# supernomad/quantum

Measured on AMD Instinct MI355X. Metric: AES-256-GCM seal+unseal GiB/s (device-resident packets) at 1/2/4/8 MI355X, higher is better.
Workload: dtype u8

## Files before the change

### quantum_amd/csrc/gcm_kernels.hip

```cpp
#include <hip/hip_runtime.h>
#include <stdint.h>

#include <algorithm>

#include "gcm_internal.h"

namespace qgcm {

typedef __attribute__((address_space(3))) uint32_t lds_u32;
typedef uint32_t u32x4 __attribute__((ext_vector_type(4)));
typedef __attribute__((address_space(3))) u32x4 lds_u128;

struct __attribute__((aligned(4))) W4 {
    uint32_t x, y, z, w;
};

#ifndef QGCM_NT_DATA
#define QGCM_NT_DATA 0
#endif
typedef uint32_t u32x4u __attribute__((ext_vector_type(4), aligned(4)));
__device__ __forceinline__ W4 load_block(const W4 *p) {
    if constexpr ((QGCM_NT_DATA & 1) != 0) {
        const u32x4u v = __builtin_nontemporal_load(reinterpret_cast<const u32x4u *>(p));
        return W4{v.x, v.y, v.z, v.w};
// ... 127 lines not shown
    const uint32_t t2 = xor3(t.t0(s2, 0), t.t1(s3, 1), rot16(xor3(t.t0(s0, 2), t.t1(s1, 3), k.rr6)));
    const uint32_t t3 = xor3(t.t0(s3, 0), t.t1(s0, 1), rot16(xor3(t.t0(s1, 2), t.t1(s2, 3), k.rr7)));
    c.U0 = t.t1(t1, 1) ^ rot16(xor3(t.t0(t2, 2), t.t1(t3, 3), k.rr8));
    c.U1 = xor3(t.t0(t1, 0), t.t1(t2, 1), rot16(t.t0(t3, 2))) ^ k.rk9;
    c.U2 = xor3(t.t0(t2, 0), t.t1(t3, 1), rot16(t.t1(t1, 3))) ^ k.rk10;
    c.U3 = t.t0(t3, 0) ^ rot16(xor3(t.t0(t1, 2), t.t1(t2, 3), k.rr11));
}
template <class A>
__device__ __forceinline__ void ctr_setup(Ctr &c, uint32_t n0, uint32_t n1, uint32_t n2, uint32_t ctr_hi,
                                          const Keys &k, const A &t) {
    ctr_setup(c, n0, n1, n2, ctr_hi, setup_keys(k), t);
}
__device__ __forceinline__ void ctr_setup(Ctr &c, uint32_t n0, uint32_t n1, uint32_t n2, uint32_t ctr_hi,
                                          const Keys &k, uint32_t lb) {
    ctr_setup(c, n0, n1, n2, ctr_hi, k, TT0{lb, 0});
}

template <class A, uint32_t kB>
__device__ __forceinline__ void ctr_block_t(const Ctr &c, uint32_t lo, const Keys &k, const A &t, uint32_t &s0,
                                            uint32_t &s1, uint32_t &s2, uint32_t &s3) {
    const uint32_t x = lo ^ c.x3;
    const uint32_t t0 = c.K0 ^ rot16(lds32(((x << 8) | t.lb) + kB + 128u));
    s0 = c.U0 ^ t.t0(t0, 0);
    s1 = c.U1 ^ rot16(t.t1(t0, 3));
    s2 = c.U2 ^ rot16(t.t0(t0, 2));
    s3 = c.U3 ^ t.t1(t0, 1);
#pragma unroll
    for (int r = 3; r < 14; ++r) round_full(s0, s1, s2, s3, k, r, t);
    round_last(s0, s1, s2, s3, k, t);
}
__device__ __forceinline__ void ctr_block(const Ctr &c, uint32_t lo, const Keys &k, uint32_t lb, uint32_t &s0,
                                          uint32_t &s1, uint32_t &s2, uint32_t &s3) {
    ctr_block_t<TT0, 0>(c, lo, k, TT0{lb, 0}, s0, s1, s2, s3);
}

template <bool kFence>
__device__ __forceinline__ void ghash_mul(uint32_t &y0, uint32_t &y1, uint32_t &y2, uint32_t &y3, uint32_t gb);

struct Tab2 {
    Keys kk;
    TT<0, true> t;
    __device__ __forceinline__ void setup(Ctr &c, uint32_t n0, uint32_t n1, uint32_t n2, uint32_t hi) const {
        ctr_setup(c, n0, n1, n2, hi, kk, t);
    }
    __device__ __forceinline__ void block(const Ctr &c, uint32_t lo, uint32_t &k0, uint32_t &k1, uint32_t &k2,
                                          uint32_t &k3) const {
        ctr_block_t<TT<0, true>, 0>(c, lo, kk, t, k0, k1, k2, k3);
    }
    __device__ __forceinline__ void ghash(uint32_t &y0, uint32_t &y1, uint32_t &y2, uint32_t &y3, uint32_t gb) const {
        ghash_mul<true>(y0, y1, y2, y3, gb);
    }
};

constexpr uint32_t kG5Windows = 26;
constexpr uint32_t kG5Bytes = kG5Windows * 512;

template <int kI>
__device__ __forceinline__ uint32_t g5_addr(const uint32_t (&y)[4], uint32_t mf8) {
    constexpr int p = 5 * kI, w = p >> 5, o = p & 31;
    uint32_t x;
    if constexpr (o > 27 && w < 3)
        x = __builtin_amdgcn_alignbit(y[w + 1], y[w], o - 3);
    else if constexpr (o > 3)
        x = y[w] >> (o - 3);
    else if constexpr (o < 3)
        x = y[w] << (3 - o);
    else
        x = y[w];
    return x & mf8;
}

template <int kLo, int kHi>
__device__ __forceinline__ void g5_chunk(const uint32_t (&y)[4], uint32_t mf8, uint32_t &a0, uint32_t &a1,
                                         uint32_t &a2, uint32_t &a3) {
    if constexpr (kLo < kHi) {
        if constexpr (QGCM_GH_PRIO > 0) __builtin_amdgcn_s_setprio(QGCM_GH_PRIO);
        const uint32_t x = g5_addr<kLo>(y, mf8);
        const u32x2 h0 = lds64(x + kLo * 512u), h1 = lds64(x + kLo * 512u + 256u);
        if constexpr (kLo + 1 < kHi) {
            const uint32_t x2 = g5_addr<kLo + 1>(y, mf8);
            const u32x2 l0 = lds64(x2 + (kLo + 1) * 512u), l1 = lds64(x2 + (kLo + 1) * 512u + 256u);
            if constexpr (QGCM_GH_PRIO > 0) __builtin_amdgcn_s_setprio(0);
            a0 = xor3(a0, h0.x, l0.x);
            a1 = xor3(a1, h0.y, l0.y);
            a2 = xor3(a2, h1.x, l1.x);
            a3 = xor3(a3, h1.y, l1.y);
            g5_chunk<kLo + 2, kHi>(y, mf8, a0, a1, a2, a3);
        } else {
            if constexpr (QGCM_GH_PRIO > 0) __builtin_amdgcn_s_setprio(0);
            a0 ^= h0.x;
            a1 ^= h0.y;
            a2 ^= h1.x;
            a3 ^= h1.y;
        }
    }
}

__device__ __forceinline__ void ghash_mul5(uint32_t &y0, uint32_t &y1, uint32_t &y2, uint32_t &y3, uint32_t mf8) {
    const uint32_t y[4] = {y0, y1, y2, y3};
    uint32_t a0 = 0, a1 = 0, a2 = 0, a3 = 0;
    g5_chunk<0, 7>(y, mf8, a0, a1, a2, a3);
    asm volatile("" : "+v"(a0), "+v"(a1), "+v"(a2), "+v"(a3)::"memory");
    g5_chunk<7, 13>(y, mf8, a0, a1, a2, a3);
    asm volatile("" : "+v"(a0), "+v"(a1), "+v"(a2), "+v"(a3)::"memory");
    g5_chunk<13, 20>(y, mf8, a0, a1, a2, a3);
    asm volatile("" : "+v"(a0), "+v"(a1), "+v"(a2), "+v"(a3)::"memory");
    g5_chunk<20, 26>(y, mf8, a0, a1, a2, a3);
    y0 = a0;
    y1 = a1;
    y2 = a2;
    y3 = a3;
}

__device__ __forceinline__ void g5_fill(const uint4 *__restrict__ comb4, uint32_t tid, uint32_t nthreads) {
    for (uint32_t e = tid; e < kG5Windows * 32u; e += nthreads) {
        const uint32_t i = e >> 5, v = e & 31u;
        uint4 c[5];
#pragma unroll
        for (uint32_t j = 0; j < 5; ++j) {
            const uint32_t t = 5 * i + j, tt = t < 128u ? t : 127u;
            const uint32_t vv = (((v >> j) & 1u) && t < 128u) ? (1u << (tt & 3u)) : 0u;
            c[j] = comb4[16u * (2u * (tt >> 3) + ((tt & 7u) < 4u ? 1u : 0u)) + vv];
        }
        uint32_t a0 = 0, a1 = 0, a2 = 0, a3 = 0;
#pragma unroll
        for (uint32_t j = 0; j < 5; ++j) {
            a0 ^= c[j].x;
            a1 ^= c[j].y;
            a2 ^= c[j].z;
            a3 ^= c[j].w;
        }
        *(lds_u64 *)(size_t)(512u * i + 8u * v) = u32x2{a0, a1};
        *(lds_u64 *)(size_t)(512u * i + 256u + 8u * v) = u32x2{a2, a3};
    }
}

struct Tab2F {
    Keys kk;
    TT<kG5Bytes, true> t;
    uint32_t mf8;
    __device__ __forceinline__ void setup(Ctr &c, uint32_t n0, uint32_t n1, uint32_t n2, uint32_t hi) const {
        ctr_setup(c, n0, n1, n2, hi, kk, t);
    }
    __device__ __forceinline__ void block(const Ctr &c, uint32_t lo, uint32_t &k0, uint32_t &k1, uint32_t &k2,
                                          uint32_t &k3) const {
        ctr_block_t<TT<kG5Bytes, true>, kG5Bytes>(c, lo, kk, t, k0, k1, k2, k3);
    }
    __device__ __forceinline__ void ghash(uint32_t &y0, uint32_t &y1, uint32_t &y2, uint32_t &y3, uint32_t) const {
        ghash_mul5(y0, y1, y2, y3, mf8);
    }
};

__device__ __forceinline__ uint32_t vreg(uint32_t x) {
    asm volatile("" : "+v"(x));
    return x;
}

template <bool kFence = true>
__device__ __forceinline__ void ghash_mul(uint32_t &y0, uint32_t &y1, uint32_t &y2, uint32_t &y3, uint32_t gb) {
    uint32_t a0 = 0, a1 = 0, a2 = 0, a3 = 0;
    const uint32_t yw[4] = {y0, y1, y2, y3};
#pragma unroll
    for (int w = 0; w < 4; ++w) {
        const uint32_t hi = yw[w] & 0xf0f0f0f0u;
        const uint32_t lo = (yw[w] << 4) & 0xf0f0f0f0u;
#pragma unroll
        for (int k = 0; k < 4; ++k) {
            const int j = 4 * w + k;
            const uint4 th = lds128(perm(gb, hi, 0x0c060500u | k) + (2 * j) * 256);
            const uint4 tl = lds128(perm(gb, lo, 0x0c060500u | k) + (2 * j + 1) * 256);
            a0 = xor3(a0, th.x, tl.x);
            a1 = xor3(a1, th.y, tl.y);
            a2 = xor3(a2, th.z, tl.z);
            a3 = xor3(a3, th.w, tl.w);
        }
        if constexpr (kFence) asm volatile("" : "+v"(a0), "+v"(a1), "+v"(a2), "+v"(a3)::"memory");
    }
    y0 = a0;
    y1 = a1;
    y2 = a2;
    y3 = a3;
}

__device__ __forceinline__ void ghash_mul_global(uint32_t &y0, uint32_t &y1, uint32_t &y2, uint32_t &y3,
                                                 const uint4 *__restrict__ T) {
    uint32_t a0 = 0, a1 = 0, a2 = 0, a3 = 0;
    const uint32_t yw[4] = {y0, y1, y2, y3};
    const char *base = reinterpret_cast<const char *>(T);
#pragma unroll
    for (int w = 0; w < 4; ++w) {
#pragma unroll
        for (int k = 0; k < 4; ++k) {
            const int j = 4 * w + k;
            const uint32_t oh = (yw[w] >> (8 * k)) & 0xf0u;
            const uint32_t ol = ((yw[w] >> (8 * k)) & 0x0fu) << 4;
            const uint4 th = *reinterpret_cast<const uint4 *>(base + (2 * j) * 256 + oh);
            const uint4 tl = *reinterpret_cast<const uint4 *>(base + (2 * j + 1) * 256 + ol);
            a0 = xor3(a0, th.x, tl.x);
            a1 = xor3(a1, th.y, tl.y);
            a2 = xor3(a2, th.z, tl.z);
            a3 = xor3(a3, th.w, tl.w);
        }
        asm volatile("" : "+v"(a0), "+v"(a1), "+v"(a2), "+v"(a3)::"memory");
    }
    y0 = a0;
    y1 = a1;
    y2 = a2;
    y3 = a3;
}

__device__ __forceinline__ void ghash_lenblock_global(uint32_t aad_len, uint32_t L, const uint4 *__restrict__ T,
                                                      uint32_t &y0, uint32_t &y1, uint32_t &y2, uint32_t &y3) {
    const char *base = reinterpret_cast<const char *>(T);
    const uint32_t w1 = bswap(aad_len * 8u), w3 = bswap(L * 8u);
    const uint32_t v[5] = {w1 >> 24, w3, w3 >> 8, w3 >> 16, w3 >> 24};
    const int j[5] = {7, 12, 13, 14, 15};
    uint32_t a0 = 0, a1 = 0, a2 = 0, a3 = 0;
#pragma unroll
    for (int i = 0; i < 5; ++i) {
        const uint4 th = *reinterpret_cast<const uint4 *>(base + (2 * j[i]) * 256 + (v[i] & 0xf0u));
        const uint4 tl = *reinterpret_cast<const uint4 *>(base + (2 * j[i] + 1) * 256 + ((v[i] & 0x0fu) << 4));
        a0 = xor3(a0, th.x, tl.x);
        a1 = xor3(a1, th.y, tl.y);
        a2 = xor3(a2, th.z, tl.z);
        a3 = xor3(a3, th.w, tl.w);
    }
    y0 = a0;
    y1 = a1;
    y2 = a2;
    y3 = a3;
}

__device__ __forceinline__ uint32_t sel4(uint32_t q, uint32_t a, uint32_t b, uint32_t c, uint32_t d) {
    return q == 0 ? a : (q == 1 ? b : (q == 2 ? c : d));
}
__device__ __forceinline__ uint32_t lowmask(uint32_t s) { return s ? (0xffffffffu >> (32 - 8 * s)) : 0u; }
__device__ __forceinline__ void store_bytes(uint8_t *p, uint32_t v, uint32_t nbytes) {
    if (nbytes > 0) p[0] = (uint8_t)v;
    if (nbytes > 1) p[1] = (uint8_t)(v >> 8);
    if (nbytes > 2) p[2] = (uint8_t)(v >> 16);
}
__device__ __forceinline__ uint32_t load_bytes(const uint8_t *p, uint32_t nbytes) {
    uint32_t v = 0;
    if (nbytes > 0) v |= p[0];
    if (nbytes > 1) v |= (uint32_t)p[1] << 8;
    if (nbytes > 2) v |= (uint32_t)p[2] << 16;
    return v;
}


__device__ __forceinline__ void read_tail(const uint8_t *data, uint32_t L, uint32_t &g0, uint32_t &g1, uint32_t &g2,
                                          uint32_t &g3, uint32_t &n0, uint32_t &n1, uint32_t &n2) {
    const uint32_t s = L & 3u;
    const uint32_t *t = reinterpret_cast<const uint32_t *>(data + (L & ~3u));
    const uint32_t w0 = t[0], w1 = t[1], w2 = t[2], w3 = t[3], w4 = t[4], w5 = t[5], w6 = t[6];
    const uint32_t w7 = load_bytes(data + (L & ~3u) + 28, s);
    g0 = __builtin_amdgcn_alignbyte(w1, w0, s);
    g1 = __builtin_amdgcn_alignbyte(w2, w1, s);
    g2 = __builtin_amdgcn_alignbyte(w3, w2, s);
    g3 = __builtin_amdgcn_alignbyte(w4, w3, s);
    n0 = __builtin_amdgcn_alignbyte(w5, w4, s);
    n1 = __builtin_amdgcn_alignbyte(w6, w5, s);
    n2 = __builtin_amdgcn_alignbyte(w7, w6, s);
}

__device__ __forceinline__ void read_nonce(const uint8_t *data, uint32_t L, uint32_t &n0, uint32_t &n1, uint32_t &n2) {
    const uint32_t s = L & 3u;
    const uint32_t *t = reinterpret_cast<const uint32_t *>(data + (L & ~3u));
    const uint32_t w4 = t[4], w5 = t[5], w6 = t[6];
    const uint32_t w7 = load_bytes(data + (L & ~3u) + 28, s);
    n0 = __builtin_amdgcn_alignbyte(w5, w4, s);
    n1 = __builtin_amdgcn_alignbyte(w6, w5, s);
    n2 = __builtin_amdgcn_alignbyte(w7, w6, s);
}
__device__ __forceinline__ void read_tag(const uint8_t *data, uint32_t L, uint32_t &g0, uint32_t &g1, uint32_t &g2,
                                         uint32_t &g3) {
    const uint32_t s = L & 3u;
    const uint32_t *t = reinterpret_cast<const uint32_t *>(data + (L & ~3u));
    const uint32_t w0 = t[0], w1 = t[1], w2 = t[2], w3 = t[3], w4 = t[4];
    g0 = __builtin_amdgcn_alignbyte(w1, w0, s);
    g1 = __builtin_amdgcn_alignbyte(w2, w1, s);
    g2 = __builtin_amdgcn_alignbyte(w3, w2, s);
    g3 = __builtin_amdgcn_alignbyte(w4, w3, s);
}

__device__ __forceinline__ uint32_t funnel(uint32_t hi, uint32_t lo, uint32_t sh) {
    return (uint32_t)((((uint64_t)hi << 32) | lo) >> sh);
}
__device__ __forceinline__ void write_tail(uint8_t *data, uint32_t L, uint32_t g0, uint32_t g1, uint32_t g2,
                                           uint32_t g3, uint32_t n0, uint32_t n1, uint32_t n2, uint32_t prefix) {
    const uint32_t s = L & 3u;
    uint32_t *t = reinterpret_cast<uint32_t *>(data + (L & ~3u));
    const uint32_t sh = 32 - 8 * s;
    t[0] = (uint32_t)((((uint64_t)g0 << 32) | ((uint64_t)prefix << sh)) >> sh);
    t[1] = funnel(g1, g0, sh);
    t[2] = funnel(g2, g1, sh);
    t[3] = funnel(g3, g2, sh);
    t[4] = funnel(n0, g3, sh);
    t[5] = funnel(n1, n0, sh);
    t[6] = funnel(n2, n1, sh);
    if (s) store_bytes(data + (L & ~3u) + 28, n2 >> sh, s);
}

__device__ __forceinline__ uint32_t quad_xor(uint32_t v) {
    v ^= (uint32_t)__builtin_amdgcn_mov_dpp((int)v, 0xB1, 0xf, 0xf, false);
    v ^= (uint32_t)__builtin_amdgcn_mov_dpp((int)v, 0x4E, 0xf, 0xf, false);
    return v;
}

template <bool kSeal, class Eng>
__device__ __forceinline__ void quad_packet(const Batch &b, const Eng &eng, uint32_t pkt, uint64_t off, uint32_t L,
                                            uint32_t wkey, uint32_t m, uint32_t gH4) {
    const uint4 *Hg = b.gh_table + (size_t)wkey * kGhEntries;
    uint8_t *raw = b.arena + off;
    uint8_t *data = raw + 4;

    uint32_t g0 = 0, g1 = 0, g2 = 0, g3 = 0, n0, n1, n2;
    if (kSeal && b.nonces) {
        const uint32_t *np = reinterpret_cast<const uint32_t *>(b.nonces + 12ull * pkt);
        n0 = np[0];
        n1 = np[1];
        n2 = np[2];
    } else {
        read_nonce(data, L, n0, n1, n2);
    }
    const uint32_t nfull = L >> 4, r = L & 15u;
    const uint32_t d = nfull + (r ? 1u : 0u);

    uint32_t z0 = 0, z1 = 0, z2 = 0, z3 = 0;
    if (m == 3 && b.aad_len)
        z0 = *reinterpret_cast<const uint32_t *>(raw) & (b.aad_len >= 4 ? 0xffffffffu : lowmask(b.aad_len));
    int blast = -1;

    uint32_t e0 = 0, e1 = 0, e2 = 0, e3 = 0;
    uint32_t prefix = 0;
    {
    Ctr cc;
    uint32_t hi = 0;
    eng.setup(cc, n0, n1, n2, 0);
    for (uint32_t bi = m; bi < nfull; bi += 4) {
        const uint32_t ctr = bi + 2;
        if ((ctr >> 8) != hi) {
            hi = ctr >> 8;
            eng.setup(cc, n0, n1, n2, hi);
        }
        W4 *p = reinterpret_cast<W4 *>(data + 16u * bi);
        const W4 in = load_block(p);
        uint32_t k0, k1, k2, k3;
        eng.block(cc, ctr & 0xffu, k0, k1, k2, k3);
        const W4 out = {in.x ^ k0, in.y ^ k1, in.z ^ k2, in.w ^ k3};
        store_block(p, out);
        const W4 &c = kSeal ? out : in;
        eng.ghash(z0, z1, z2, z3, gH4);
        z0 ^= c.x;
        z1 ^= c.y;
        z2 ^= c.z;
        z3 ^= c.w;
        blast = (int)bi;
    }
    const bool part = r && (nfull & 3u) == m;
    if (part || m == (d & 3u)) {
        const uint32_t ctr = part ? nfull + 2 : 1u;
        if ((ctr >> 8) != hi) {
            hi = ctr >> 8;
            eng.setup(cc, n0, n1, n2, hi);
        }
        uint32_t k0, k1, k2, k3;
        eng.block(cc, ctr & 0xffu, k0, k1, k2, k3);
        if (part) {
            uint8_t *blk = data + 16u * nfull;
            const W4 in = *reinterpret_cast<const W4 *>(blk);
            const uint32_t q = r >> 2, sb = r & 3u;
            const uint32_t o0 = in.x ^ k0, o1 = in.y ^ k1, o2 = in.z ^ k2, o3 = in.w ^ k3;
            uint32_t *bw = reinterpret_cast<uint32_t *>(blk);
            if (q > 0) bw[0] = o0;
            if (q > 1) bw[1] = o1;
            if (q > 2) bw[2] = o2;
            const uint32_t oq = sel4(q, o0, o1, o2, o3) & lowmask(sb);
            W4 c = kSeal ? W4{o0, o1, o2, o3} : in;
            if (kSeal)
                prefix = oq;
            else
                store_bytes(blk + 4 * q, oq, sb);
            c.x &= q > 0 ? 0xffffffffu : lowmask(sb);
            c.y &= q > 1 ? 0xffffffffu : (q == 1 ? lowmask(sb) : 0u);
            c.z &= q > 2 ? 0xffffffffu : (q == 2 ? lowmask(sb) : 0u);
            c.w &= q == 3 ? lowmask(sb) : 0u;
            eng.ghash(z0, z1, z2, z3, gH4);
            z0 ^= c.x;
            z1 ^= c.y;
            z2 ^= c.z;
            z3 ^= c.w;
            blast = (int)nfull;
        } else {
            e0 = k0;
            e1 = k1;
            e2 = k2;
            e3 = k3;
        }
    }
    }
    {
        const uint32_t em = d + 1u - (uint32_t)blast;
        const uint32_t tsel = em == 2 ? kGhH2 : em == 3 ? kGhH3 : em == 4 ? kGhH4 : kGhH5;
        ghash_mul_global(z0, z1, z2, z3, Hg + tsel);
        uint32_t l0, l1, l2, l3;
        ghash_lenblock_global(b.aad_len, L, Hg, l0, l1, l2, l3);
        z0 = quad_xor(z0) ^ l0;
        z1 = quad_xor(z1) ^ l1;
        z2 = quad_xor(z2) ^ l2;
        z3 = quad_xor(z3) ^ l3;
    }
    e0 = quad_xor(e0);
    e1 = quad_xor(e1);
    e2 = quad_xor(e2);
    e3 = quad_xor(e3);
    const uint32_t t0 = z0 ^ e0, t1 = z1 ^ e1, t2 = z2 ^ e2, t3 = z3 ^ e3;
    const uint32_t owner = r ? (nfull & 3u) : 0u;
    if (kSeal) {
        if (m == owner) {
            write_tail(data, L, t0, t1, t2, t3, n0, n1, n2, prefix);
            if (b.status) b.status[pkt] = 1;
        }
    } else {
        read_tag(data, L, g0, g1, g2, g3);
        const bool ok = ((t0 ^ g0) | (t1 ^ g1) | (t2 ^ g2) | (t3 ^ g3)) == 0;
        if (!ok) {
            for (uint32_t bi = m; bi < nfull; bi += 4) {
                const W4 zz = {0, 0, 0, 0};
                *reinterpret_cast<W4 *>(data + 16u * bi) = zz;
            }
            if (r && m == owner) {
                uint32_t *bw = reinterpret_cast<uint32_t *>(data + 16u * nfull);
                for (uint32_t w = 0; w < (r >> 2); ++w) bw[w] = 0;
                store_bytes(data + 16u * nfull + (r & ~3u), 0, r & 3u);
            }
        }
        if (b.status && m == 0) b.status[pkt] = ok ? 1 : 0;
    }
}

#ifndef QGCM_TILE_POOL
#define QGCM_TILE_POOL 4
#endif
#ifndef QGCM_TAIL_EIGHTHS
#define QGCM_TAIL_EIGHTHS 4
#endif
constexpr uint32_t kPoolCtr = kG5Bytes + kTeBytes;

#ifdef QGCM_QUAD_STATS
__device__ unsigned long long g_quad_stats[4096 * 8];
#endif

template <bool kDesc>
constexpr int quad_waves() { return kDesc ? 12 : 16; }
template <bool kDesc>
constexpr int quad_wpe() { return kDesc ? 3 : 8; }

template <bool kSeal, bool kDesc>
__global__ void __launch_bounds__(quad_waves<kDesc>() * 64) __attribute__((amdgpu_waves_per_eu(quad_wpe<kDesc>(),
                                                                                                  quad_wpe<kDesc>())))
gcm_quad_kernel(Batch b, const uint32_t *__restrict__ rk_table) {
    constexpr uint32_t kW = quad_waves<kDesc>();
    constexpr uint32_t kT = kW * 64;
    constexpr uint32_t kTeBase = kDesc ? 0u : kG5Bytes;
    const uint32_t lane = threadIdx.x & 63u;
    const uint32_t wave = threadIdx.x >> 6;
    const uint32_t m = lane & 3u;
    const uint32_t qd = lane >> 2;
    if (kDesc && b.tile_list && __builtin_amdgcn_readfirstlane(*b.n_list) == 0) return;

    for (uint32_t i = threadIdx.x; i < kTeBytes / 4; i += kT) {
        const uint32_t x = i >> 6, slot = i & 63u;
        lds_st32(kTeBase + 4 * i, b.te[(slot >> 5) * 256u + x]);
    }
    if constexpr (!kDesc) g5_fill(b.gh_table + (size_t)b.uniform_key * kGhEntries + kGhH4, threadIdx.x, kT);
    if constexpr (!kDesc && QGCM_TILE_POOL) {
        if (threadIdx.x == 0) lds_st32(kPoolCtr, kW);
    }
#if QGCM_TILE_POOL == 4
    if constexpr (!kDesc) {
        if (threadIdx.x == 0) lds_st32(kPoolCtr + 12, 0u);
    }
#endif
    __syncthreads();

    const uint32_t lb = (lane & 31u) << 2;
    const uint32_t m8 = vreg(0x0000ff00u), mf8 = vreg(0x000000f8u);
    const uint32_t gH4 = kDesc ? kTeBytes + wave * kGhBytes : 0u;
    uint32_t cur_key = kDesc ? 0xffffffffu : b.uniform_key;
    const uint32_t ntiles = kDesc ? (b.tile_list ? *b.n_list : b.n_items >> 4) : ((b.n + 15) >> 4);

#ifdef QGCM_QUAD_STATS
    unsigned long long *qs = g_quad_stats + (size_t)blockIdx.x * 8u;
    uint32_t qs_tiles = 0;
    if (!kDesc && threadIdx.x == 0) {
        qs[0] = wall_clock64();
        qs[4] = __builtin_amdgcn_s_getreg((31 << 11) | 20);
        qs[5] = __builtin_amdgcn_s_getreg((31 << 11) | 4);
    }
#endif
#ifdef QGCM_QUAD_STATS
#define QS_TILE() ++qs_tiles
#define QS_END()                                                  \
    do {                                                          \
        if (!kDesc && lane == 0) {                                \
            const unsigned long long t_ = wall_clock64();         \
            atomicMax(&qs[1], t_);                                \
            atomicAdd(&qs[2], t_);                                \
            atomicAdd(&qs[3], (unsigned long long)qs_tiles);      \
            atomicMax(&qs[6], (1ull << 62) - t_);                 \
        }                                                         \
    } while (0)
#else
#define QS_TILE() do { } while (0)
#define QS_END() do { } while (0)
#endif
#if QGCM_TILE_POOL == 4
    uint32_t sidx = 0xffffffffu, tail0 = 0;
    if constexpr (!kDesc) {
        const uint32_t rows = ntiles / (gridDim.x * kW);
        if (b.pool && rows > 0) {
            const uint32_t tail_rows = rows < 2 ? 0u : std::min(rows - 1u, std::max(1u, rows * QGCM_TAIL_EIGHTHS / 8u));
            sidx = (rows - tail_rows) * kW;
            tail0 = (rows - tail_rows) * gridDim.x * kW;
        }
    }
#endif
    uint32_t tile = blockIdx.x * kW + wave;
    if constexpr (kDesc) {
        uint32_t t = 0;
        if (lane == 0) t = atomicAdd(b.tile_counter, 1u);
        tile = __builtin_amdgcn_readfirstlane(__shfl(t, 0));
    }
    for (; tile < ntiles;) {
        uint32_t pkt, L;
        bool valid;
        uint64_t off;
        uint32_t wkey = cur_key;
        if constexpr (kDesc) {
            const uint32_t wt = b.tile_list ? b.tile_list[tile] : tile;
            pkt = b.worklist[wt * 16u + qd];
            valid = pkt != 0xffffffffu;
            qgcm_desc dsc = {0, 0, 0};
            if (valid) dsc = b.descs[pkt];
            off = dsc.offset;
            L = kSeal ? dsc.len : dsc.len - QGCM_OVERHEAD;
            const uint64_t vmask = __ballot(valid);
            if (vmask != 0) {
                wkey = __builtin_amdgcn_readfirstlane(__shfl(dsc.key_idx, __ffsll((unsigned long long)vmask) - 1));
                if (wkey != cur_key) {
                    const uint4 *src = b.gh_table + (size_t)wkey * kGhEntries + kGhH4;
#pragma unroll
                    for (int r = 0; r < 8; ++r) {
                        const uint32_t e = r * 64 + lane;
                        lds_st_comb(gH4, e, src[e]);
                    }
                    __builtin_amdgcn_fence(__ATOMIC_RELEASE, "wavefront");
                    __builtin_amdgcn_wave_barrier();
                    __builtin_amdgcn_fence(__ATOMIC_ACQUIRE, "wavefront");
                    cur_key = wkey;
                }
            }
            uint32_t t = 0;
            if (lane == 0) t = atomicAdd(b.tile_counter, 1u);
            const uint32_t next = __builtin_amdgcn_readfirstlane(__shfl(t, 0));
            asm volatile("" : "+v"(L));
            if (!valid) {
                tile = next;
                continue;
            }
            tile = next;
        } else {
            pkt = tile * 16u + qd;
            L = b.uniform_len;
            asm volatile("" : "+s"(L));
            valid = pkt < b.n;
            if (!kSeal) {
                if (L < (uint32_t)QGCM_OVERHEAD) valid = false;
                L -= QGCM_OVERHEAD;
            }
            off = (uint64_t)pkt * b.stride;
            if constexpr (QGCM_TILE_POOL) {
                uint32_t i = 0;
                if (lane == 0) i = __atomic_fetch_add((lds_u32 *)(size_t)kPoolCtr, 1u, __ATOMIC_RELAXED);
                i = __builtin_amdgcn_readfirstlane(i);
                tile = blockIdx.x * kW + (i % kW) + (i / kW) * gridDim.x * kW;
#if QGCM_TILE_POOL == 4
                if (i >= sidx) {
                    uint32_t c = 0;
                    if (lane == 0) c = atomicAdd(b.pool, 1u);
                    tile = tail0 + __builtin_amdgcn_readfirstlane(c);
                }
#endif
            } else {
                tile += gridDim.x * kW;
            }
            if (!valid) {
                if (!kSeal && b.status && pkt < b.n && m == 0) b.status[pkt] = 0;
                continue;
            }
        }
        const Keys kk = {rk_table + (size_t)wkey * kRkWords, rk_table + (size_t)wkey * kRkWords + 64};
        if constexpr (kDesc) {
            quad_packet<kSeal>(b, Tab2{kk, {lb, m8}}, pkt, off, L, wkey, m, gH4);
        } else {
            quad_packet<kSeal>(b, Tab2F{kk, {lb, m8}, mf8}, pkt, off, L, wkey, m, gH4);
        }
        QS_TILE();
    }
    QS_END();
#if QGCM_TILE_POOL == 4
    if constexpr (!kDesc) {
        if (b.pool) {
            uint32_t last = 0;
            if (lane == 0 && __atomic_fetch_add((lds_u32 *)(size_t)(kPoolCtr + 12), 1u, __ATOMIC_RELAXED) == kW - 1) {
                __threadfence();
                last = atomicAdd(b.pool + kPoolDoneWord, 1u) == gridDim.x - 1u ? 1u : 0u;
            }
            if (lane == 0 && last) {
                __threadfence();
                b.pool[0] = 0;
                b.pool[kPoolDoneWord] = 0;
                __threadfence_system();
                __hip_atomic_store(b.pool_done, b.pool_gen, __ATOMIC_RELEASE, __HIP_MEMORY_SCOPE_SYSTEM);
            }
        }
    }
#endif
}
#undef QS_TILE
#undef QS_END

#ifdef QGCM_QUAD_STATS
extern "C" int qgcm_debug_quad_stats(unsigned long long *out, int n, int reset) {
    if (n > 4096 * 8) n = 4096 * 8;
    if (hipMemcpyFromSymbol(out, HIP_SYMBOL(g_quad_stats), (size_t)n * 8) != hipSuccess) return -1;
    if (reset) {
        static unsigned long long zero[4096 * 8];
        if (hipMemcpyToSymbol(HIP_SYMBOL(g_quad_stats), zero, sizeof(zero)) != hipSuccess) return -1;
    }
    return 0;
}
#endif

constexpr uint32_t kSegCtl = kG5Bytes + kTeBytes;
constexpr uint32_t kSegLds = kSegCtl + 16u;
constexpr uint32_t kSegDone = 0xffffffffu;

__device__ __forceinline__ volatile lds_u32 *seg_ctl(uint32_t i) { return (volatile lds_u32 *)(size_t)(kSegCtl + 4u * i); }

template <class P>
__device__ __forceinline__ uint32_t wave_lower_bound(uint32_t lo, uint32_t hi, uint32_t lane, P pred) {
    while (hi - lo > 63u) {
        const uint32_t step = (hi - lo + 62u) / 63u;
        const uint32_t p = min(lo + lane * step, hi);
        const uint64_t msk = __ballot(pred(p));
        const uint32_t f = (uint32_t)__ffsll((unsigned long long)msk) - 1u;
        if (f == 0) return lo;
        const uint32_t nlo = lo + (f - 1u) * step + 1u, nhi = min(lo + f * step, hi);
        lo = nlo;
        hi = nhi;
    }
    const uint64_t msk = __ballot(pred(min(lo + lane, hi)));
    return lo + (uint32_t)__ffsll((unsigned long long)msk) - 1u;
}

#ifdef QGCM_SEG_STATS
__device__ unsigned long long g_seg_stats[4096 * 16];
#define SEG_STAT_ADD(i, v) \
    do { if (lane == 0) atomicAdd(&g_seg_stats[blockIdx.x * 16u + (i)], (unsigned long long)(v)); } while (0)
#define SEG_NOW() wall_clock64()
#else
#define SEG_STAT_ADD(i, v) do { } while (0)
#define SEG_NOW() 0ull
#endif

#ifndef QGCM_SEG_START
#define QGCM_SEG_START 1
#endif
#ifndef QGCM_SEG_HELP_MIN
#define QGCM_SEG_HELP_MIN 16
#endif
#ifndef QGCM_SEG_LAST
#define QGCM_SEG_LAST 0
#endif
__device__ __forceinline__ void seg_next_phase(const Batch &b, uint32_t &r, uint32_t nruns, bool &helping,
                                               uint32_t lane) {
    uint32_t found = kSegDone;
    if (!helping) {
        uint32_t c = 0;
        if (lane == 0) c = atomicAdd(b.tile_counter, 1u);
        c = __builtin_amdgcn_readfirstlane(__shfl(c, 0));
        if (c < nruns)
            found = c;
        else
            helping = true;
    }
    if (helping) {
        if (QGCM_SEG_START) {
            const uint32_t h = (blockIdx.x * 0x9E3779B1u) ^ (r * 0x85EBCA6Bu + 0x632BE5ABu);
            r = (uint32_t)(((uint64_t)(h ^ (h >> 15)) * nruns) >> 32);
        }
        for (uint32_t pass = 0, need = QGCM_SEG_HELP_MIN; pass < (QGCM_SEG_LAST ? 2u : 1u) && found == kSegDone;
             ++pass, need = QGCM_SEG_LAST ? QGCM_SEG_LAST : 1u)
        for (uint32_t base = 0; base < nruns; base += 256u) {
            bool left[4];
            uint32_t idx[4];
#pragma unroll
            for (uint32_t j = 0; j < 4; ++j) {
                const uint32_t o = base + 64u * j + lane;
                uint32_t i = r + o;
                i = i >= nruns ? i - nruns : i;
                idx[j] = i;
                left[j] = false;
                if (o < nruns) {
                    const uint2 run = b.runs[i];
                    left[j] = __hip_atomic_load(b.run_next + i, __ATOMIC_RELAXED, __HIP_MEMORY_SCOPE_AGENT) +
                                  need <= run.y - run.x;
                }
            }
#pragma unroll
            for (uint32_t j = 0; j < 4 && found == kSegDone; ++j) {
                const uint64_t msk = __ballot(left[j]);
                if (msk) found = __builtin_amdgcn_readfirstlane(__shfl(idx[j], (int)__ffsll((unsigned long long)msk) - 1));
            }
            if (found != kSegDone) break;
        }
    }
    uint32_t key = kSegDone;
    if (found != kSegDone) {
        r = found;
        key = b.tile_keys[b.runs[found].x];
    }
    if (lane == 0) {
        *seg_ctl(0) = found;
        *seg_ctl(1) = key;
    }
}

#ifndef QGCM_SEG_CLAIM
#define QGCM_SEG_CLAIM 1
#endif

template <bool kSeal>
__global__ void __launch_bounds__(1024) __attribute__((amdgpu_waves_per_eu(8, 8)))
gcm_seg_kernel(Batch b, const uint32_t *__restrict__ rk_table) {
    constexpr uint32_t kT = 1024;
    const uint32_t lane = threadIdx.x & 63u;
    const uint32_t wave = threadIdx.x >> 6;
    const uint32_t m = lane & 3u;
    const uint32_t qd = lane >> 2;
    if (__builtin_amdgcn_readfirstlane(*b.nruns) == 0) return;
    for (uint32_t i = threadIdx.x; i < kTeBytes / 4; i += kT) {
        const uint32_t x = i >> 6, slot = i & 63u;
        lds_st32(kG5Bytes + 4 * i, b.te[(slot >> 5) * 256u + x]);
    }
    const uint32_t lb = (lane & 31u) << 2;
    const uint32_t m8 = vreg(0x0000ff00u), mf8 = vreg(0x000000f8u);
    const uint32_t ntiles = b.n_items >> 4;
    uint32_t table_key = kSegDone;
    uint32_t r = 0, nruns = 0;
    bool helping = false;
    if (wave == 0) {
        nruns = *b.nruns;
        const uint32_t t = (uint32_t)((uint64_t)ntiles * blockIdx.x / gridDim.x);
        const uint32_t i = wave_lower_bound(0u, nruns, lane, [&](uint32_t j) { return j == nruns || b.runs[j].x > t; });
        r = i ? i - 1u : 0u;
        SEG_STAT_ADD(6, r);
        SEG_STAT_ADD(8, __builtin_amdgcn_s_getreg((31 << 11) | 20));
        SEG_STAT_ADD(9, __builtin_amdgcn_s_getreg((31 << 11) | 4));
    }
    __syncthreads();
    [[maybe_unused]] unsigned long long t_idle = SEG_NOW();
    if (wave == 0) SEG_STAT_ADD(2, t_idle);
    [[maybe_unused]] uint32_t ntile_stat = 0;
    for (;;) {
        if (wave == 0) {
            [[maybe_unused]] const unsigned long long t0 = SEG_NOW();
            seg_next_phase(b, r, nruns, helping, lane);
            SEG_STAT_ADD(7, SEG_NOW() - t0);
        }
        __syncthreads();
        if (wave == 0) SEG_STAT_ADD(0, 1);
        const uint32_t run = __builtin_amdgcn_readfirstlane(*seg_ctl(0));
        const uint32_t key = __builtin_amdgcn_readfirstlane(*seg_ctl(1));
        if (run == kSegDone) break;
        if (key != table_key) {
            g5_fill(b.gh_table + (size_t)key * kGhEntries + kGhH4, threadIdx.x, kT);
            table_key = key;
            __syncthreads();
        }
        [[maybe_unused]] const unsigned long long t_busy = SEG_NOW();
        SEG_STAT_ADD(4, t_busy - t_idle);
        const uint2 rt = b.runs[run];
        const Tab2F e3 = {{rk_table + (size_t)key * kRkWords, rk_table + (size_t)key * kRkWords + 64}, {lb, m8}, mf8};
        for (uint32_t t = 0, left = 0;; ++t, --left) {
            if (left == 0) {
                uint32_t nx = 0;
                if (lane == 0) nx = atomicAdd(b.run_next + run, (uint32_t)QGCM_SEG_CLAIM);
                t = rt.x + __builtin_amdgcn_readfirstlane(__shfl(nx, 0));
                left = QGCM_SEG_CLAIM;
            }
            if (t >= rt.y) break;
            const uint32_t pkt = b.worklist[t * 16u + qd];
            if (pkt != 0xffffffffu) {
                const qgcm_desc dsc = b.descs[pkt];
                const uint32_t L = kSeal ? dsc.len : dsc.len - QGCM_OVERHEAD;
                quad_packet<kSeal, Tab2F>(b, e3, pkt, dsc.offset, L, key, m, 0u);
            }
            ++ntile_stat;
        }
        t_idle = SEG_NOW();
        SEG_STAT_ADD(5, t_idle - t_busy);
        __syncthreads();
    }
    SEG_STAT_ADD(1, ntile_stat);
    if (wave == 0) SEG_STAT_ADD(3, SEG_NOW());
}

#ifdef QGCM_SEG_STATS
extern "C" int qgcm_debug_seg_stats(unsigned long long *out, int n, int reset) {
    if (n > 4096 * 16) n = 4096 * 16;
    if (hipMemcpyFromSymbol(out, HIP_SYMBOL(g_seg_stats), (size_t)n * 8) != hipSuccess) return -1;
    if (reset) {
        static unsigned long long zero[4096 * 16];
        if (hipMemcpyToSymbol(HIP_SYMBOL(g_seg_stats), zero, sizeof(zero)) != hipSuccess) return -1;
    }
    return 0;
}
#endif

constexpr uint32_t kOneThreads = 512;
constexpr uint32_t kOneTabs = 7;
constexpr uint32_t kOneBuf = kTeBytes + kOneTabs * kGhBytes;
constexpr uint32_t kOneScratch = kOneBuf + kOneCap;
constexpr uint32_t kOneX = kOneScratch + 64;
constexpr uint32_t kOneLds = kOneX + 2048;
constexpr uint32_t kOneSliceMax = kOneThreads / 4;
static_assert(kOneLds <= 160u * 1024u, "gfx950 LDS is 160 KiB per workgroup");
#ifdef QGCM_RES_TRACE
constexpr uint32_t kResTrace = ((kOneLds + 15u) & ~15u) + 16;
__device__ __forceinline__ void res_stamp(uint32_t slot, uint32_t by = 0) {
    if (threadIdx.x == by) {
        const uint64_t t = wall_clock64();
        lds_st32(kResTrace + 8 * slot, (uint32_t)t);
        lds_st32(kResTrace + 8 * slot + 4, (uint32_t)(t >> 32));
    }
}
#endif

typedef __attribute__((address_space(3))) uint8_t lds_u8;
__device__ __forceinline__ uint32_t lds8(uint32_t addr) { return *(const lds_u8 *)(size_t)addr; }
__device__ __forceinline__ void lds_st8(uint32_t addr, uint32_t v) { *(lds_u8 *)(size_t)addr = (uint8_t)v; }
__device__ __forceinline__ uint32_t lds32u(uint32_t a) {
    return lds8(a) | lds8(a + 1) << 8 | lds8(a + 2) << 16 | lds8(a + 3) << 24;
}
__device__ __forceinline__ void lds_st32u(uint32_t a, uint32_t v) {
    lds_st8(a, v);
    lds_st8(a + 1, v >> 8);
    lds_st8(a + 2, v >> 16);
    lds_st8(a + 3, v >> 24);
}
__device__ __forceinline__ void block_mask(uint32_t r, uint32_t &m0, uint32_t &m1, uint32_t &m2, uint32_t &m3) {
    const uint32_t q = r >> 2, sb = r & 3u;
    m0 = q > 0 ? 0xffffffffu : lowmask(sb);
    m1 = q > 1 ? 0xffffffffu : (q == 1 ? lowmask(sb) : 0u);
    m2 = q > 2 ? 0xffffffffu : (q == 2 ? lowmask(sb) : 0u);
    m3 = q == 3 ? lowmask(sb) : 0u;
}

constexpr int kSc0Sc1 = 1 | 16;
__device__ __forceinline__ uint4 host_ld16(const void *base, uint32_t bytes, uint32_t off) {
    const __amdgpu_buffer_rsrc_t r = __builtin_amdgcn_make_buffer_rsrc(const_cast<void *>(base), 0, (int)bytes, 0x00020000);
    const u32x4 v = __builtin_amdgcn_raw_buffer_load_b128(r, (int)off, 0, kSc0Sc1);
    return uint4{v.x, v.y, v.z, v.w};
}
__device__ __forceinline__ void host_st16(void *base, uint32_t bytes, uint32_t off, uint4 v) {
    const __amdgpu_buffer_rsrc_t r = __builtin_amdgcn_make_buffer_rsrc(base, 0, (int)bytes, 0x00020000);
    __builtin_amdgcn_raw_buffer_store_b128(u32x4{v.x, v.y, v.z, v.w}, r, (int)off, 0, kSc0Sc1);
}

template <bool kSys>
__device__ __forceinline__ uint4 slot_ld16(const uint8_t *slot, uint32_t i) {
    if constexpr (kSys) return host_ld16(slot, kResSlotBytes, 16 * i);
    return reinterpret_cast<const uint4 *>(slot)[i];
}
template <bool kSys>
__device__ __forceinline__ void slot_st16(uint8_t *slot, uint32_t i, uint4 v) {
    if constexpr (kSys) {
        host_st16(slot, kResSlotBytes, 16 * i, v);
        return;
    }
    reinterpret_cast<uint4 *>(slot)[i] = v;
}
template <bool kSys>
__device__ __forceinline__ void slot_st16_at(uint8_t *slot, uint32_t off, uint4 v) {
    const __amdgpu_buffer_rsrc_t r =
        __builtin_amdgcn_make_buffer_rsrc(slot, 0, (int)(kSys ? kResSlotBytes : kOneCap), 0x00020000);
    __builtin_amdgcn_raw_buffer_store_b128(u32x4{v.x, v.y, v.z, v.w}, r, (int)off, 0, kSys ? kSc0Sc1 : 0);
}

__device__ __forceinline__ void ghash_mul8(uint32_t &z0, uint32_t &z1, uint32_t &z2, uint32_t &z3, uint32_t gb,
                                           uint32_t e) {
    const uint32_t w = e >> 1, k0 = 2u * (e & 1u);
    const uint32_t y = w == 0 ? z0 : w == 1 ? z1 : w == 2 ? z2 : z3;
    const uint32_t hi = y & 0xf0f0f0f0u, lo = (y << 4) & 0xf0f0f0f0u;
    const uint32_t r0 = gb + 1024u * e;
    const uint4 t0 = lds128(r0 + ((hi >> (8 * k0)) & 0xffu));
    const uint4 t1 = lds128(r0 + 256u + ((lo >> (8 * k0)) & 0xffu));
// ... 1126 lines not shown
```

Measured before the change: 854.2.

## Carry unfinished GCM tail work across consecutive uniform tiles to balance quad lanes

```diff
diff --git a/quantum_amd/csrc/gcm_kernels.hip b/quantum_amd/csrc/gcm_kernels.hip
--- a/quantum_amd/csrc/gcm_kernels.hip
+++ b/quantum_amd/csrc/gcm_kernels.hip
@@ -453,20 +453,20 @@
     if (s) store_bytes(data + (L & ~3u) + 28, n2 >> sh, s);
 }
 
+__device__ __forceinline__ uint32_t lane_again() {
+    uint32_t t = threadIdx.x;
+    asm volatile("" : "+v"(t));
+    return t & 63u;
+}
 __device__ __forceinline__ uint32_t quad_xor(uint32_t v) {
     v ^= (uint32_t)__builtin_amdgcn_mov_dpp((int)v, 0xB1, 0xf, 0xf, false);
     v ^= (uint32_t)__builtin_amdgcn_mov_dpp((int)v, 0x4E, 0xf, 0xf, false);
     return v;
 }
 
-template <bool kSeal, class Eng>
-__device__ __forceinline__ void quad_packet(const Batch &b, const Eng &eng, uint32_t pkt, uint64_t off, uint32_t L,
-                                            uint32_t wkey, uint32_t m, uint32_t gH4) {
-    const uint4 *Hg = b.gh_table + (size_t)wkey * kGhEntries;
-    uint8_t *raw = b.arena + off;
-    uint8_t *data = raw + 4;
-
-    uint32_t g0 = 0, g1 = 0, g2 = 0, g3 = 0, n0, n1, n2;
+template <bool kSeal>
+__device__ __forceinline__ void load_nonce(const Batch &b, const uint8_t *data, uint32_t pkt, uint32_t L,
+                                           uint32_t &n0, uint32_t &n1, uint32_t &n2) {
     if (kSeal && b.nonces) {
         const uint32_t *np = reinterpret_cast<const uint32_t *>(b.nonces + 12ull * pkt);
         n0 = np[0];
@@ -475,6 +475,59 @@
     } else {
         read_nonce(data, L, n0, n1, n2);
     }
+}
+
+#ifndef QGCM_TILE_CARRY
+#define QGCM_TILE_CARRY 1
+#endif
+constexpr uint32_t kCarryNone = 0, kCarryDefer = 1, kCarryTake = 2;
+
+template <bool kSeal>
+__device__ __forceinline__ void partial_block(uint8_t *blk, uint32_t r, uint32_t k0, uint32_t k1, uint32_t k2,
+                                              uint32_t k3, uint32_t &prefix, W4 &c) {
+    const W4 in = *reinterpret_cast<const W4 *>(blk);
+    const uint32_t q = r >> 2, sb = r & 3u;
+    const uint32_t o0 = in.x ^ k0, o1 = in.y ^ k1, o2 = in.z ^ k2, o3 = in.w ^ k3;
+    uint32_t *bw = reinterpret_cast<uint32_t *>(blk);
+    if (q > 0) bw[0] = o0;
+    if (q > 1) bw[1] = o1;
+    if (q > 2) bw[2] = o2;
+    const uint32_t oq = sel4(q, o0, o1, o2, o3) & lowmask(sb);
+    c = kSeal ? W4{o0, o1, o2, o3} : in;
+    if (kSeal)
+        prefix = oq;
+    else
+        store_bytes(blk + 4 * q, oq, sb);
+    c.x &= q > 0 ? 0xffffffffu : lowmask(sb);
+    c.y &= q > 1 ? 0xffffffffu : (q == 1 ? lowmask(sb) : 0u);
+    c.z &= q > 2 ? 0xffffffffu : (q == 2 ? lowmask(sb) : 0u);
+    c.w &= q == 3 ? lowmask(sb) : 0u;
+}
+
+template <bool kOpaque>
+__device__ __forceinline__ void zero_plain(uint8_t *data, uint32_t nfull, uint32_t r, uint32_t m, uint32_t owner) {
+    for (uint32_t bi = m; bi < nfull; bi += 4) {
+        const uint32_t zero = kOpaque ? vreg(0u) : 0u;
+        const W4 zz = {zero, zero, zero, zero};
+        *reinterpret_cast<W4 *>(data + 16u * bi) = zz;
+    }
+    if (r && m == owner) {
+        uint32_t *bw = reinterpret_cast<uint32_t *>(data + 16u * nfull);
+        for (uint32_t w = 0; w < (r >> 2); ++w) bw[w] = 0;
+        store_bytes(data + 16u * nfull + (r & ~3u), 0, r & 3u);
+    }
+}
+
+template <bool kSeal, class Eng, bool kCarry = false>
+__device__ __forceinline__ void quad_packet(const Batch &b, const Eng &eng, uint32_t pkt, uint64_t off, uint32_t L,
+                                            uint32_t wkey, uint32_t m, uint32_t gH4, uint32_t mode, uint32_t tile,
+                                            uint32_t tile_a, uint32_t &c0, uint32_t &c1, uint32_t &c2, uint32_t &c3) {
+    const uint4 *Hg = b.gh_table + (size_t)wkey * kGhEntries;
+    uint8_t *raw = b.arena + off;
+    uint8_t *data = raw + 4;
+
+    uint32_t g0 = 0, g1 = 0, g2 = 0, g3 = 0, n0, n1, n2;
+    load_nonce<kSeal>(b, data, pkt, L, n0, n1, n2);
     const uint32_t nfull = L >> 4, r = L & 15u;
     const uint32_t d = nfull + (r ? 1u : 0u);
 
@@ -491,7 +544,13 @@
     eng.setup(cc, n0, n1, n2, 0);
     for (uint32_t bi = m; bi < nfull; bi += 4) {
         const uint32_t ctr = bi + 2;
-        if ((ctr >> 8) != hi) {
+        if constexpr (kCarry) {
+            if (ctr >= 256u && (ctr & 0xfcu) == 0) {
+                asm volatile("" ::: "memory");
+                load_nonce<kSeal>(b, data, tile * 16u + (lane_again() >> 2), L, n0, n1, n2);
+                eng.setup(cc, n0, n1, n2, ctr >> 8);
+            }
+        } else if ((ctr >> 8) != hi) {
             hi = ctr >> 8;
             eng.setup(cc, n0, n1, n2, hi);
         }
@@ -507,36 +566,139 @@
         z1 ^= c.y;
         z2 ^= c.z;
         z3 ^= c.w;
-        blast = (int)bi;
-    }
+        if constexpr (!kCarry) blast = (int)bi;
+    }
+    if constexpr (kCarry) {
+        const uint32_t ln = lane_again();
+        m = ln & 3u;
+        pkt = tile * 16u + (ln >> 2);
+        const uint32_t cnt = (nfull + 3u - m) >> 2;
+        blast = cnt ? (int)(m + 4u * cnt - 4u) : -1;
+        hi = cnt ? (uint32_t)(blast + 2) >> 8 : 0u;
+        const uint32_t p = nfull & 3u;
+        uint32_t rel = (m - p) & 3u;
+        if (mode == kCarryDefer) {
+            uint32_t l0, l1, l2, l3;
+            ghash_lenblock_global(b.aad_len, L, Hg, l0, l1, l2, l3);
+            c0 = (uint32_t)__builtin_amdgcn_mov_dpp((int)z0, 0x4E, 0xf, 0xf, false);
+            c1 = (uint32_t)__builtin_amdgcn_mov_dpp((int)z1, 0x4E, 0xf, 0xf, false);
+            c2 = (uint32_t)__builtin_amdgcn_mov_dpp((int)z2, 0x4E, 0xf, 0xf, false);
+            c3 = (uint32_t)__builtin_amdgcn_mov_dpp((int)z3, 0x4E, 0xf, 0xf, false);
+            c0 = rel == 2 ? c0 : (rel & 1u) ? l0 : 0u;
+            c1 = rel == 2 ? c1 : (rel & 1u) ? l1 : 0u;
+            c2 = rel == 2 ? c2 : (rel & 1u) ? l2 : 0u;
+            c3 = rel == 2 ? c3 : (rel & 1u) ? l3 : 0u;
+            asm volatile("" : "+v"(c0), "+v"(c1), "+v"(c2), "+v"(c3)::"memory");
+            const uint32_t em = d + 1u - (uint32_t)blast;
+            const uint32_t tsel = em == 3 ? kGhH3 : em == 4 ? kGhH4 : kGhH5;
+            ghash_mul_global(z0, z1, z2, z3, Hg + tsel);
+            z0 = quad_xor(rel ? z0 : 0u);
+            z1 = quad_xor(rel ? z1 : 0u);
+            z2 = quad_xor(rel ? z2 : 0u);
+            z3 = quad_xor(rel ? z3 : 0u);
+            c0 ^= rel == 3 ? z0 : 0u;
+            c1 ^= rel == 3 ? z1 : 0u;
+            c2 ^= rel == 3 ? z2 : 0u;
+            c3 ^= rel == 3 ? z3 : 0u;
+            return;
+        }
+        if (mode == kCarryTake) {
+            bool isa = rel >= 2, j0 = (rel & 1u) != 0;
+            uint32_t pkt_a = tile_a * 16u + (ln >> 2), pktx = isa ? pkt_a : pkt;
+            uint8_t *data_a = b.arena + (uint64_t)pkt_a * b.stride + 4;
+            uint8_t *datax = isa ? data_a : data;
+            load_nonce<kSeal>(b, datax, pktx, L, n0, n1, n2);
+            const uint32_t ctr = j0 ? 1u : nfull + 2;
+            eng.setup(cc, n0, n1, n2, ctr >> 8);
+            uint32_t k0, k1, k2, k3;
+            eng.block(cc, ctr & 0xffu, k0, k1, k2, k3);
+            uint32_t v0 = (uint32_t)__builtin_amdgcn_mov_dpp((int)z0, 0x93, 0xf, 0xf, false);
+            uint32_t v1 = (uint32_t)__builtin_amdgcn_mov_dpp((int)z1, 0x93, 0xf, 0xf, false);
+            uint32_t v2 = (uint32_t)__builtin_amdgcn_mov_dpp((int)z2, 0x93, 0xf, 0xf, false);
+            uint32_t v3 = (uint32_t)__builtin_amdgcn_mov_dpp((int)z3, 0x93, 0xf, 0xf, false);
+            uint32_t x0 = rel == 2 ? c0 : rel == 3 ? v0 : z0;
+            uint32_t x1 = rel == 2 ? c1 : rel == 3 ? v1 : z1;
+            uint32_t x2 = rel == 2 ? c2 : rel == 3 ? v2 : z2;
+            uint32_t x3 = rel == 2 ? c3 : rel == 3 ? v3 : z3;
+            W4 cm = {0, 0, 0, 0};
+            if (!j0) partial_block<kSeal>(datax + 16u * nfull, r, k0, k1, k2, k3, prefix, cm);
+            c0 = j0 ? c0 ^ k0 : 0u;
+            c1 = j0 ? c1 ^ k1 : 0u;
+            c2 = j0 ? c2 ^ k2 : 0u;
+            c3 = j0 ? c3 ^ k3 : 0u;
+            eng.ghash(x0, x1, x2, x3, gH4);
+            x0 ^= cm.x;
+            x1 ^= cm.y;
+            x2 ^= cm.z;
+            x3 ^= cm.w;
+            v0 = (uint32_t)__builtin_amdgcn_mov_dpp((int)x0, 0x39, 0xf, 0xf, false);
+            v1 = (uint32_t)__builtin_amdgcn_mov_dpp((int)x1, 0x39, 0xf, 0xf, false);
+            v2 = (uint32_t)__builtin_amdgcn_mov_dpp((int)x2, 0x39, 0xf, 0xf, false);
+            v3 = (uint32_t)__builtin_amdgcn_mov_dpp((int)x3, 0x39, 0xf, 0xf, false);
+            c0 = rel == 2 ? v0 : c0;
+            c1 = rel == 2 ? v1 : c1;
+            c2 = rel == 2 ? v2 : c2;
+            c3 = rel == 2 ? v3 : c3;
+            uint32_t y0 = rel == 3 ? z0 : x0, y1 = rel == 3 ? z1 : x1;
+            uint32_t y2 = rel == 3 ? z2 : x2, y3 = rel == 3 ? z3 : x3;
+            const uint32_t tsel = rel == 1 ? kGhH : rel == 3 ? kGhH3 : kGhH2;
+            ghash_mul_global(y0, y1, y2, y3, Hg + tsel);
+            {
+                const uint32_t l2 = lane_again();
+                m = l2 & 3u;
+                rel = (m - p) & 3u;
+                isa = rel >= 2;
+                j0 = (rel & 1u) != 0;
+                pkt = tile * 16u + (l2 >> 2);
+                pkt_a = tile_a * 16u + (l2 >> 2);
+                pktx = isa ? pkt_a : pkt;
+                data = b.arena + (uint64_t)pkt * b.stride + 4;
+                data_a = b.arena + (uint64_t)pkt_a * b.stride + 4;
+                datax = isa ? data_a : data;
+            }
+            const uint32_t tb0 = quad_xor(rel == 2 ? c0 : rel == 1 ? y0 ^ c0 : y0);
+            const uint32_t tb1 = quad_xor(rel == 2 ? c1 : rel == 1 ? y1 ^ c1 : y1);
+            const uint32_t tb2 = quad_xor(rel == 2 ? c2 : rel == 1 ? y2 ^ c2 : y2);
+            const uint32_t tb3 = quad_xor(rel == 2 ? c3 : rel == 1 ? y3 ^ c3 : y3);
+            const uint32_t ta0 = quad_xor(rel == 2 ? y0 : rel == 3 ? c0 : 0u);
+            const uint32_t ta1 = quad_xor(rel == 2 ? y1 : rel == 3 ? c1 : 0u);
+            const uint32_t ta2 = quad_xor(rel == 2 ? y2 : rel == 3 ? c2 : 0u);
+            const uint32_t ta3 = quad_xor(rel == 2 ? y3 : rel == 3 ? c3 : 0u);
+            const uint32_t t0 = isa ? ta0 : tb0, t1 = isa ? ta1 : tb1, t2 = isa ? ta2 : tb2, t3 = isa ? ta3 : tb3;
+            if (kSeal) {
+                if (!j0) {
+                    load_nonce<kSeal>(b, datax, pktx, L, n0, n1, n2);
+                    write_tail(datax, L, t0, t1, t2, t3, n0, n1, n2, prefix);
+                    if (b.status) b.status[pktx] = 1;
+                }
+            } else {
+                read_tag(datax, L, g0, g1, g2, g3);
+                const uint32_t bad = ((t0 ^ g0) | (t1 ^ g1) | (t2 ^ g2) | (t3 ^ g3)) != 0 ? 1u : 0u;
+                const uint32_t bad_b = quad_xor(rel == 0 ? bad : 0u), bad_a = quad_xor(rel == 2 ? bad : 0u);
+                if (bad_b) zero_plain<true>(data, nfull, r, m, p);
+                if (bad_a) zero_plain<true>(data_a, nfull, r, m, p);
+                if (b.status && m == 0) {
+                    b.status[pkt] = bad_b ? 0 : 1;
+                    b.status[pkt_a] = bad_a ? 0 : 1;
+                }
+            }
+            return;
+        }
+    }
+    if constexpr (kCarry) c0 = c1 = c2 = c3 = 0;
     const bool part = r && (nfull & 3u) == m;
     if (part || m == (d & 3u)) {
         const uint32_t ctr = part ? nfull + 2 : 1u;
         if ((ctr >> 8) != hi) {
             hi = ctr >> 8;
+            if constexpr (kCarry) load_nonce<kSeal>(b, data, pkt, L, n0, n1, n2);
             eng.setup(cc, n0, n1, n2, hi);
         }
         uint32_t k0, k1, k2, k3;
         eng.block(cc, ctr & 0xffu, k0, k1, k2, k3);
         if (part) {
-            uint8_t *blk = data + 16u * nfull;
-            const W4 in = *reinterpret_cast<const W4 *>(blk);
-            const uint32_t q = r >> 2, sb = r & 3u;
-            const uint32_t o0 = in.x ^ k0, o1 = in.y ^ k1, o2 = in.z ^ k2, o3 = in.w ^ k3;
-            uint32_t *bw = reinterpret_cast<uint32_t *>(blk);
-            if (q > 0) bw[0] = o0;
-            if (q > 1) bw[1] = o1;
-            if (q > 2) bw[2] = o2;
-            const uint32_t oq = sel4(q, o0, o1, o2, o3) & lowmask(sb);
-            W4 c = kSeal ? W4{o0, o1, o2, o3} : in;
-            if (kSeal)
-                prefix = oq;
-            else
-                store_bytes(blk + 4 * q, oq, sb);
-            c.x &= q > 0 ? 0xffffffffu : lowmask(sb);
-            c.y &= q > 1 ? 0xffffffffu : (q == 1 ? lowmask(sb) : 0u);
-            c.z &= q > 2 ? 0xffffffffu : (q == 2 ? lowmask(sb) : 0u);
-            c.w &= q == 3 ? lowmask(sb) : 0u;
+            W4 c;
+            partial_block<kSeal>(data + 16u * nfull, r, k0, k1, k2, k3, prefix, c);
             eng.ghash(z0, z1, z2, z3, gH4);
             z0 ^= c.x;
             z1 ^= c.y;
@@ -557,6 +719,7 @@
         ghash_mul_global(z0, z1, z2, z3, Hg + tsel);
         uint32_t l0, l1, l2, l3;
         ghash_lenblock_global(b.aad_len, L, Hg, l0, l1, l2, l3);
+        if constexpr (kCarry) asm volatile("" : "+v"(l0), "+v"(l1), "+v"(l2), "+v"(l3)::"memory");
         z0 = quad_xor(z0) ^ l0;
         z1 = quad_xor(z1) ^ l1;
         z2 = quad_xor(z2) ^ l2;
@@ -570,25 +733,22 @@
     const uint32_t owner = r ? (nfull & 3u) : 0u;
     if (kSeal) {
         if (m == owner) {
+            if constexpr (kCarry) load_nonce<kSeal>(b, data, pkt, L, n0, n1, n2);
             write_tail(data, L, t0, t1, t2, t3, n0, n1, n2, prefix);
             if (b.status) b.status[pkt] = 1;
         }
     } else {
         read_tag(data, L, g0, g1, g2, g3);
         const bool ok = ((t0 ^ g0) | (t1 ^ g1) | (t2 ^ g2) | (t3 ^ g3)) == 0;
-        if (!ok) {
-            for (uint32_t bi = m; bi < nfull; bi += 4) {
-                const W4 zz = {0, 0, 0, 0};
-                *reinterpret_cast<W4 *>(data + 16u * bi) = zz;
-            }
-            if (r && m == owner) {
-                uint32_t *bw = reinterpret_cast<uint32_t *>(data + 16u * nfull);
-                for (uint32_t w = 0; w < (r >> 2); ++w) bw[w] = 0;
-                store_bytes(data + 16u * nfull + (r & ~3u), 0, r & 3u);
-            }
-        }
+        if (!ok) zero_plain<kCarry>(data, nfull, r, m, owner);
         if (b.status && m == 0) b.status[pkt] = ok ? 1 : 0;
     }
+}
+template <bool kSeal, class Eng>
+__device__ __forceinline__ void quad_packet(const Batch &b, const Eng &eng, uint32_t pkt, uint64_t off, uint32_t L,
+                                            uint32_t wkey, uint32_t m, uint32_t gH4) {
+    uint32_t c0 = 0, c1 = 0, c2 = 0, c3 = 0;
+    quad_packet<kSeal, Eng, false>(b, eng, pkt, off, L, wkey, m, gH4, kCarryNone, 0u, 0u, c0, c1, c2, c3);
 }
 
 #ifndef QGCM_TILE_POOL
@@ -684,11 +844,15 @@
         if (lane == 0) t = atomicAdd(b.tile_counter, 1u);
         tile = __builtin_amdgcn_readfirstlane(__shfl(t, 0));
     }
+    constexpr uint32_t kNoCarry = 0xffffffffu;
+    uint32_t carry_tile = kNoCarry, c0 = 0, c1 = 0, c2 = 0, c3 = 0;
     for (; tile < ntiles;) {
         uint32_t pkt, L;
         bool valid;
         uint64_t off;
         uint32_t wkey = cur_key;
+        uint32_t mode = kCarryNone, pm = m;
+        const uint32_t cur = tile;
         if constexpr (kDesc) {
             const uint32_t wt = b.tile_list ? b.tile_list[tile] : tile;
             pkt = b.worklist[wt * 16u + qd];
@@ -723,7 +887,10 @@
             }
             tile = next;
         } else {
-            pkt = tile * 16u + qd;
+            const uint32_t tl = QGCM_TILE_CARRY != 0 ? lane_again() : lane;
+            const uint32_t tqd = tl >> 2;
+            pm = tl & 3u;
+            pkt = tile * 16u + tqd;
             L = b.uniform_len;
             asm volatile("" : "+s"(L));
             valid = pkt < b.n;
@@ -734,13 +901,13 @@
             off = (uint64_t)pkt * b.stride;
             if constexpr (QGCM_TILE_POOL) {
                 uint32_t i = 0;
-                if (lane == 0) i = __atomic_fetch_add((lds_u32 *)(size_t)kPoolCtr, 1u, __ATOMIC_RELAXED);
+                if (tl == 0) i = __atomic_fetch_add((lds_u32 *)(size_t)kPoolCtr, 1u, __ATOMIC_RELAXED);
                 i = __builtin_amdgcn_readfirstlane(i);
                 tile = blockIdx.x * kW + (i % kW) + (i / kW) * gridDim.x * kW;
 #if QGCM_TILE_POOL == 4
                 if (i >= sidx) {
                     uint32_t c = 0;
-                    if (lane == 0) c = atomicAdd(b.pool, 1u);
+                    if (tl == 0) c = atomicAdd(b.pool, 1u);
                     tile = tail0 + __builtin_amdgcn_readfirstlane(c);
                 }
 #endif
@@ -748,15 +915,26 @@
                 tile += gridDim.x * kW;
             }
             if (!valid) {
-                if (!kSeal && b.status && pkt < b.n && m == 0) b.status[pkt] = 0;
+                if (!kSeal && b.status && pkt < b.n && pm == 0) b.status[pkt] = 0;
                 continue;
+            }
+            if constexpr (QGCM_TILE_CARRY != 0) {
+                const uint32_t nf = L >> 4, whole = b.n >> 4;
+                if (carry_tile != kNoCarry)
+                    mode = kCarryTake;
+                else if ((L & 15u) != 0 && nf != 0 && ((nf + 1u) & 2u) == 0 && cur < whole && tile < whole)
+                    mode = kCarryDefer;
             }
         }
         const Keys kk = {rk_table + (size_t)wkey * kRkWords, rk_table + (size_t)wkey * kRkWords + 64};
         if constexpr (kDesc) {
-            quad_packet<kSeal>(b, Tab2{kk, {lb, m8}}, pkt, off, L, wkey, m, gH4);
+            quad_packet<kSeal>(b, Tab2{kk, {lb, m8}}, pkt, off, L, wkey, pm, gH4);
+        } else if constexpr (QGCM_TILE_CARRY != 0) {
+            quad_packet<kSeal, Tab2F, true>(b, Tab2F{kk, {lb, m8}, mf8}, pkt, off, L, wkey, pm, gH4, mode,
+                                            cur, carry_tile, c0, c1, c2, c3);
+            carry_tile = mode == kCarryDefer ? cur : kNoCarry;
         } else {
-            quad_packet<kSeal>(b, Tab2F{kk, {lb, m8}, mf8}, pkt, off, L, wkey, m, gH4);
+            quad_packet<kSeal>(b, Tab2F{kk, {lb, m8}, mf8}, pkt, off, L, wkey, pm, gH4);
         }
         QS_TILE();
     }
```

Result: no change. 861.5, median of 6 (+0.9%).
